# federicomegler/sq-learn

Measured on AMD Instinct MI355X. Metric: q-means fit samples/sec (Lloyd samples*iterations/s, delta-means + tomography noise), higher is better.
Workload: dtype fp32; 1 GPU; model=q-means k=1024 delta=0.5 (10000000 x 256 synthetic), global_batch=10000000, seq_len=256, parallelism=dp1

## Files before the change

sq_learn_amd/csrc/estep_f32.hip:

```cpp
#include "common.h"
#include "band.h"
#include "f16_tile.h"
#include "sq_api.h"

namespace sq {

constexpr int kMaxCand = 16;

#ifndef SQ_SPLIT_ACC_ALL
#define SQ_SPLIT_ACC_ALL 1
#endif
template <int KSD, int TOP = 2>
__global__ void __launch_bounds__(256, 1) estep_f32_kernel(
    const float* __restrict__ X, const _Float16* __restrict__ C, const float* __restrict__ xn,
    int* __restrict__ labels, float* __restrict__ mind, long long* __restrict__ ovf_rows,
    int* __restrict__ ovf_count, double* __restrict__ part, long long n, int k_pad, float alpha,
    float inv_alpha2, float delta_s, RngKey key, long long row_offset, int ovf_cap,
    const long long* __restrict__ rlist, const int* __restrict__ rcount,
    const float* __restrict__ cmax2_p, long long* __restrict__ mrows, int* __restrict__ mcand,
    int* __restrict__ multi_count, unsigned char* __restrict__ xflag, long long mcap) {
  const float Cm = cmax2_p ? sqrtf(*cmax2_p) * (1.0f + 0x1p-16f) : 0.0f;
  constexpr bool SPLIT_ACC = SQ_SPLIT_ACC_ALL || TOP == 3;
  constexpr float kEps3 =
      SPLIT_ACC ? (3.0f * 0x1p-22f + (KSD * 16 + 18.0f) * 0x1p-24f + 2.0f * KSD * 16 * 0x1p-34f) *
// ... 386 lines not shown
constexpr int kStampWaves = 8192;
constexpr int kStampN = 12;
__device__ unsigned long long g_x64_stamps[kStampWaves * kStampN];
#define SQ_STAMP_NOW() __builtin_amdgcn_s_memtime()
#endif

template <int KSD>
using X64Ring = TileRing<KSD, kX64Waves>;

template <int KSD>
struct X64RowSets {
  static constexpr int value = KSD <= 16 ? 2 : 1;
};
constexpr int kX64Pfd = 2;

template <int KSD, int RS>
__global__ void __launch_bounds__(kX64Waves * 64) estep_x64_kernel(
    const _Float16* __restrict__ Xh, const float* __restrict__ X, const _Float16* __restrict__ C,
    const float* __restrict__ Cm, const float* __restrict__ xn, const float* __restrict__ cmax2_p,
    int* __restrict__ labels, float* __restrict__ mind, long long* __restrict__ dense_rows,
    int* __restrict__ dense_count, long long* __restrict__ mrows, int* __restrict__ mcand,
    int* __restrict__ multi_count, long long n, int k_pad, float alpha, float delta_s,
    RngKey key, long long row_offset, int dense_cap, int qbits, const long long* __restrict__ rlist,
    const int* __restrict__ rcount, float* __restrict__ ub, float* __restrict__ lb,
    int* __restrict__ mflag) {
  constexpr int NW = kX64Waves;
  constexpr int DX = KSD * 16;
  using Ring = X64Ring<KSD>;
  constexpr int KT = Ring::KT, NS = Ring::NS, SK = Ring::SK, RING = Ring::RING;
  constexpr int ROWS = NW * 32 * RS;
  extern __shared__ __attribute__((aligned(16))) unsigned char smem[];
  auto buf = [&](int g) -> unsigned char* { return Ring::buf(smem, g); };
  int* cand_all = reinterpret_cast<int*>(smem + Ring::BYTES);
  int* cnt_all = cand_all + NW * RS * 32 * kMaxCand;

  const int tid = threadIdx.x;
  const int lane = tid & 63;
  const int wave = __builtin_amdgcn_readfirstlane(tid >> 6);
  const int r32 = lane & 31;
  const int half = lane >> 5;
  const int n_tiles = k_pad / kTileN;
  const long long ne = rlist ? min((long long)*rcount, n) : n;
  auto row_at = [&](long long pos) -> long long {
    const long long q = pos < ne ? pos : ne - 1;
    return rlist ? rlist[q] : q;
  };
  const long long nblk = (ne + ROWS - 1) / ROWS;
  long long blk = blockIdx.x;
  if (blk >= nblk) return;
  const uint32_t qmask = (1u << qbits) - 1u;
  const uint32_t keep = ~qmask;
  const float Ch = 2.0f * sqrtf(*cmax2_p) * (1.0f + 0x1p-16f);
  const float pack_rel = ldexpf(1.0f, qbits - 23) + 0x1p-15f;
  const float sub_rel = 0x1p-21f * sqrtf((float)DX);

  auto stage = [&](int U) { Ring::stage(C, smem, U, n_tiles); };

  f16x8 ah[RS][KSD];
  auto load_a = [&](long long b) {
    sq::load_a(ah, half, [&](int st) {
      return Xh + (size_t)row_at(b * ROWS + (wave * RS + st) * 32 + r32) * DX;
    });
  };
  const f16x8 aug = aug_frag(half);
  const int rl_own = acc_row(r32 >> 1, half);
  float xn_cur[RS], xn_nxt[RS];
  auto load_xn = [&](long long b, float (&dst)[RS]) {
#pragma unroll
    for (int st = 0; st < RS; ++st) dst[st] = xn[row_at(b * ROWS + (wave * RS + st) * 32 + rl_own)];
  };

  float m1[RS][16], m2[RS][16], m3[RS][16];
  const int lane_off = f16op::lane_off(half, r32);
  auto ins = [&](int st, int i, float v, uint32_t q) {
    const float p = and_or(v, keep, q);
    const float a1 = m1[st][i], a2 = m2[st][i];
    m3[st][i] = vmed3(a2, p, m3[st][i]);
    m2[st][i] = vmed3(a1, p, a2);
    m1[st][i] = vmin(a1, p);
  };
  typedef f32x16 Acc[RS][2];
  auto sub_step = [&](auto S_, const unsigned char* cur, Acc& acc, const Acc& o, int t_prev,
                      bool do_epi) {
    constexpr int S = decltype(S_)::value;
// ... 55 lines not shown
#endif
  };

  int U = 0;
  auto tile = [&](Acc& acc, const Acc& o, int t_prev, bool do_epi) {
#pragma unroll
    for (int st = 0; st < RS; ++st) acc[st][0] = acc[st][1] = (f32x16){0};
    static_for<NS>([&](auto S_) {
      stage(U + RING - 1);
      sub_step(S_, buf(U), acc, o, t_prev, do_epi);
      sync_tile();
      ++U;
    });
  };

  stage(0);
  stage(1);
  load_a(blk);
  load_xn(blk, xn_cur);
  asm volatile("s_waitcnt vmcnt(0)" ::: "memory");
  __builtin_amdgcn_s_barrier();

  for (; blk < nblk; blk += gridDim.x) {
#pragma unroll
    for (int st = 0; st < RS; ++st)
#pragma unroll
      for (int i = 0; i < 16; ++i) m1[st][i] = m2[st][i] = m3[st][i] = __builtin_inff();
    if constexpr (RS == 1) {
      Acc pA, pB;
      tile(pA, pA, 0, false);
      int t = 0;
      while (true) {
        if (t + 1 >= n_tiles) {
          load_a(blk + gridDim.x);
          load_xn(blk + gridDim.x, xn_nxt);
          epi_all(pA, t);
          break;
        }
        tile(pB, pA, t, true);
        ++t;
        if (t + 1 >= n_tiles) {
          load_a(blk + gridDim.x);
          load_xn(blk + gridDim.x, xn_nxt);
          epi_all(pB, t);
          break;
        }
        tile(pA, pB, t, true);
        ++t;
      }
    } else {
      f32x16 cA[RS], cB[RS];
      constexpr int PFD = kX64Pfd;
      f16x8 bq[PFD + 1];
      static_assert(NS == 1, "row sets need whole tiles per LDS slot");
#if SQ_X64_STAMP
      const unsigned long long sw0 = SQ_STAMP_NOW();
      st_first = true;
      ++st_blocks;
#endif
      for (int t = 0; t < n_tiles; ++t) {
#if SQ_X64_STAMP
        const unsigned long long sg0 = SQ_STAMP_NOW();
#endif
        stage(U + RING - 1);
#if SQ_X64_STAMP
        st_stage += SQ_STAMP_NOW() - sg0;
#endif
        tile_prime<KT>(buf(U), lane_off, bq);
        half_pass<0>(buf(U), lane_off, ah, aug, bq, cA, cB, (uint32_t)(2 * t - 1), t > 0, ins);
        half_pass<1>(buf(U), lane_off, ah, aug, bq, cB, cA, (uint32_t)(2 * t), true, ins);
        sync_tile();
        ++U;
      }
#if SQ_X64_STAMP
      const unsigned long long sl0 = SQ_STAMP_NOW();
#endif
      load_a(blk + gridDim.x);
      load_xn(blk + gridDim.x, xn_nxt);
#if SQ_X64_STAMP
      st_aload += SQ_STAMP_NOW() - sl0;
#endif
      half_drain(cB, (uint32_t)(2 * n_tiles - 1), ins);
#if SQ_X64_STAMP
      st_sweep += SQ_STAMP_NOW() - sw0;
#endif
    }
#if SQ_X64_STAMP
    const unsigned long long sp0 = SQ_STAMP_NOW();
#endif

#pragma nounroll
    for (int st = 0; st < RS; ++st) {
#if SQ_X64_STAMP
    const unsigned long long sc0 = SQ_STAMP_NOW();
#endif
    const long long row0 = blk * ROWS + (wave * RS + st) * 32;
    int* cand = cand_all + (wave * RS + st) * 32 * kMaxCand;
    int* cnt = cnt_all + (wave * RS + st) * 32;
    float ms1[16], ms2[16], ms3[16];
#pragma unroll
    for (int i = 0; i < 16; ++i) {
      ms1[i] = m1[0][i]; ms2[i] = m2[0][i]; ms3[i] = m3[0][i];
#pragma unroll
      for (int o = 1; o < RS; ++o) {
        const float a1 = m1[o][i], a2 = m2[o][i], a3 = m3[o][i];
        ms1[i] = st == o ? a1 : ms1[i];
        ms2[i] = st == o ? a2 : ms2[i];
        ms3[i] = st == o ? a3 : ms3[i];
      }
    }

    auto row_min = [&](float (&R)[16]) -> float {
#pragma unroll
      for (int o = 16, c = 8; o >= 2; o >>= 1, c >>= 1) {
        const bool hi = (r32 & o) != 0;
#pragma unroll
        for (int j = 0; j < c; ++j) {
          const float lo_v = R[j], hi_v = R[c + j];
          const float keepv = hi ? hi_v : lo_v, sendv = hi ? lo_v : hi_v;
          R[j] = vmin(keepv, __shfl_xor(sendv, o, 64));
        }
      }
      return vmin(R[0], __shfl_xor(R[0], 1, 64));
    };
    float R[16];
#pragma unroll
    for (int i = 0; i < 16; ++i) R[i] = ms1[i];
    const float rmin = row_min(R);
    float xn_own = xn_cur[0];
#pragma unroll
    for (int o = 1; o < RS; ++o) xn_own = st == o ? xn_cur[o] : xn_own;
    const float xsv = alpha * sqrtf(xn_own) * (1.0f + 0x1p-16f);
    const float prod = xsv * Ch;
    const float mag = 0.25f * Ch * Ch + prod;
    const float E = 1.0625f * 0x1p-10f * prod + pack_rel * mag + sub_rel * (xsv + Ch);
    const float T_own = __uint_as_float(__float_as_uint(rmin) & keep) + delta_s + 2.0f * E;

#if SQ_X64_STAMP
    const unsigned long long sc1 = SQ_STAMP_NOW();
    st_rmin += sc1 - sc0;
#endif
    float nc[16];
    float Tr[16];
#pragma unroll
    for (int i = 0; i < 16; ++i) Tr[i] = __shfl(T_own, 32 * half + 2 * i, 64);
    int* const sink = cnt_all + NW * RS * 32 + wave * 64 + lane;
#pragma unroll
    for (int i = 0; i < 16; ++i) {
      const float T = Tr[i];
      nc[i] = ms1[i] > T ? ms1[i] : (ms2[i] > T ? ms2[i] : ms3[i]);
      const int rl = acc_row(i, half);
      auto jof = [&](float p) -> int {
        const uint32_t q = __float_as_uint(p) & qmask;
        return (int)((q >> 1) * kTileN + (q & 1u) * 32u) + r32;
      };
      const unsigned long long b1 = __ballot(ms1[i] <= T), b2 = __ballot(ms2[i] <= T);
      const unsigned long long b3 = __ballot(ms3[i] <= T);
      const uint32_t b1l = (uint32_t)b1, b1h = (uint32_t)(b1 >> 32);
      const uint32_t b2l = (uint32_t)b2, b2h = (uint32_t)(b2 >> 32);
      const int c1 = __popc(half ? b1h : b1l), c2 = __popc(half ? b2h : b2l);
      const bool d3 = (half ? (uint32_t)(b3 >> 32) : (uint32_t)b3) != 0u;
      const int s1 = (int)__builtin_amdgcn_mbcnt_hi(b1h, __builtin_amdgcn_mbcnt_lo(b1l, 0u)) -
                     (half ? __popc(b1l) : 0);
      const int s2 = c1 + (int)__builtin_amdgcn_mbcnt_hi(b2h, __builtin_amdgcn_mbcnt_lo(b2l, 0u)) -
                     (half ? __popc(b2l) : 0);
      *((ms1[i] <= T && s1 < kMaxCand) ? cand + rl * kMaxCand + s1 : sink) = jof(ms1[i]);
      *((ms2[i] <= T && s2 < kMaxCand) ? cand + rl * kMaxCand + s2 : sink) = jof(ms2[i]);
      *(r32 == 0 ? cnt + rl : sink) = c1 + c2 + (d3 ? kMaxCand + 1 : 0);
    }
#if SQ_X64_STAMP
    const unsigned long long sc2 = SQ_STAMP_NOW();
    st_cl += sc2 - sc1;
#endif
    float ub_own = 0.f, lb_own = 0.f;
    if (ub) {
      const float ncmin = row_min(nc);
      const float ia2 = 1.0f / (alpha * alpha);
      const float d1 = (__uint_as_float(__float_as_uint(rmin) & keep) + E) * ia2;
      const float d2 = (__uint_as_float(__float_as_uint(ncmin) & keep) - E) * ia2;
      const float marg = 0x1p-20f * (xn_own + fabsf(d1) + fabsf(d2));
      ub_own = sqrtf(fmaxf(xn_own + d1 + marg, 0.f)) * (1.0f + 0x1p-20f);
      lb_own = sqrtf(fmaxf(xn_own + d2 - marg, 0.f)) * (1.0f - 0x1p-20f);
    }
    asm volatile("s_waitcnt lgkmcnt(0)" ::: "memory");
    __builtin_amdgcn_wave_barrier();
#if SQ_X64_STAMP
    st_cand += SQ_STAMP_NOW() - sc0;
    st_ub += SQ_STAMP_NOW() - sc2;
#endif

    const bool valid = row0 + r32 < ne;
    const long long g = row_at(row0 + r32);
    if (ub) {
      const int src = ((r32 & 3) + 4 * ((r32 >> 3) & 3)) * 2 + 32 * ((r32 >> 2) & 1);
      const float u = __shfl(ub_own, src, 64), l = __shfl(lb_own, src, 64);
      if (valid && half == 0) {
        ub[g] = u;
        lb[g] = cnt[r32] <= kMaxCand ? l : 0.0f;
      }
    }
    const int c_r = cnt[r32];
    const bool dense = c_r > kMaxCand;
    const bool multi = valid && !dense && c_r >= 2;
    if (mflag && valid && half == 0 && !multi) mflag[g] = 0;
    if (valid && half == 0) {
      if (dense) {
        const int s = atomicAdd(dense_count, 1);
        if (s < dense_cap) dense_rows[s] = g;
        labels[g] = -1;
      } else if (c_r == 1) {
        labels[g] = cand[r32 * kMaxCand];
        mind[g] = -1.0f;
      }
    }
    const bool mrow = multi && half == 0;
    const unsigned long long mm = __ballot(mrow);
    const int nm = __popcll(mm);
    int mbase = 0;
    if (lane == 0 && nm) mbase = atomicAdd(multi_count, nm);
    mbase = __shfl(mbase, 0, 64);
    if (mrow) {
      const long long slot = (long long)mbase + __popcll(mm & ((1ull << lane) - 1ull));
      if (mflag) mflag[g] = slot < n ? 1 : 0;
      if (slot < n) {
        mrows[slot] = g;
        int* mc = mcand + g * (kMaxCand + 1);
        mc[0] = c_r;
        for (int c = 0; c < c_r; ++c) mc[1 + c] = cand[r32 * kMaxCand + c];
      } else {
        const int s2 = atomicAdd(dense_count, 1);
        if (s2 < dense_cap) dense_rows[s2] = g;
        labels[g] = -1;
      }
    }
    asm volatile("s_waitcnt lgkmcnt(0)" ::: "memory");
    __builtin_amdgcn_wave_barrier();
    }
#pragma unroll
    for (int st = 0; st < RS; ++st) xn_cur[st] = xn_nxt[st];
#if SQ_X64_STAMP
    st_post += SQ_STAMP_NOW() - sp0;
#endif
  }
  asm volatile("s_waitcnt vmcnt(0)" ::: "memory");
#if SQ_X64_STAMP
  const int sidx = blockIdx.x * NW + wave;
  if (lane == 0 && sidx < kStampWaves) {
    unsigned long long* o = g_x64_stamps + (size_t)sidx * kStampN;
    o[0] = SQ_STAMP_NOW() - st_t0; o[1] = st_sweep; o[2] = st_sync; o[3] = st_sync0;
    o[4] = st_post; o[5] = st_blocks; o[6] = st_stage; o[7] = st_cand; o[8] = st_aload;
    o[9] = st_rmin; o[10] = st_cl; o[11] = st_ub;
  }
#endif
}

constexpr int kBfLdsK = 2048;
template <int PER>
// ... 1130 lines not shown
    hipOccupancyMaxActiveBlocksPerMultiprocessor(&per_cu, (const void*)gap_screen_kernel<DX>, 256,
                                                 0);
    gres = (long long)(cus > 0 ? cus : 256) * (per_cu > 0 ? per_cu : 2);
  }
  const unsigned bgrid =
      grid_blocks > 0 ? (unsigned)grid_blocks : (unsigned)min(max(rblocks, 1LL), gres);
  hipLaunchKernelGGL(gap_screen_kernel<DX>, dim3(bgrid), dim3(256), 0, st, (const _Float16*)Xh,
                     (const float*)xn, mrec.mrows_b, mrec.count_b, mrec.dsh, mrec.dsh_stride,
                     mrec.dq, mrec.dsh_stride / DX * 8, inv_alpha, delta, (int*)labels, mrec.rec,
                     mrec.mflag, mrec.it_now, mrec.ring, max(1, mrec.ring / 2), (long long*)mrows,
                     (int*)multi_count, cap, mrec.n_done, mrec.mrows_mv, mrec.count_mv,
                     (float*)ydbg);
  return (int)hipGetLastError();
}

template <int KSD>
static int launch_estep_x64(const void* Xh, const void* X, const void* C, const void* Cm,
                            const void* xn, const void* cmax2, void* labels, void* mind,
                            void* dense_rows, void* dense_count, void* mrows, void* mcand,
                            void* multi_count, void* corr, long long n, int k_pad, float alpha,
                            float delta_s, double delta, RngKey key, long long row_offset,
                            int dense_cap, hipStream_t st, const void* rlist, const void* rcount,
                            void* ub, void* lb, void* mflag, void* xflag, int list_rs,
                            const MultiRec& mrec, bool defer_rows = false) {
  int qbits = 1;
  while ((1 << qbits) < 2 * (k_pad / kTileN)) ++qbits;
  auto go = [&](auto RS_) {
    constexpr int RS = decltype(RS_)::value;
    constexpr int NW = kX64Waves;
    const size_t lds =
        (size_t)X64Ring<KSD>::BYTES + (size_t)NW * RS * 32 * (kMaxCand + 1) * 4 +
        (size_t)NW * 64 * 4;
    auto kern = estep_x64_kernel<KSD, RS>;
    static bool attr = false;
    if (!attr) {
      hipFuncSetAttribute((const void*)kern, hipFuncAttributeMaxDynamicSharedMemorySize,
                          160 * 1024);
      attr = true;
    }
    static int resident = 0;
    if (resident == 0) resident = resident_blocks((const void*)kern, NW * 64, lds);
    const long long nblk = (n + NW * 32 * RS - 1) / (NW * 32 * RS);
    const unsigned grid = (unsigned)(nblk < resident && !rlist ? nblk : resident);
    hipLaunchKernelGGL(kern, dim3(grid), dim3(NW * 64), lds, st, (const _Float16*)Xh,
                       (const float*)X, (const _Float16*)C, (const float*)Cm, (const float*)xn,
                       (const float*)cmax2, (int*)labels, (float*)mind, (long long*)dense_rows,
                       (int*)dense_count, (long long*)mrows, (int*)mcand, (int*)multi_count, n,
                       k_pad, alpha, delta_s, key, row_offset, dense_cap, qbits,
                       (const long long*)rlist, (const int*)rcount, (float*)ub, (float*)lb,
                       (int*)mflag);
  };
  static const bool list_rs1 = [] {
    const char* e = getenv("SQ_X64_LIST_RS1");
    return !(e && e[0] == '0');
  }();
  if (rlist && (list_rs == 1 || (list_rs == 0 && list_rs1)))
    go(std::integral_constant<int, 1>{});
  else
    go(std::integral_constant<int, X64RowSets<KSD>::value>{});
  int rc = (int)hipGetLastError();
  if (rc) return rc;
  const long long rblocks = (n / 16 + 63) / 64;
  const unsigned rgrid = (unsigned)(rblocks < 4096 ? (rblocks > 0 ? rblocks : 1) : 4096);
  if (xflag && mrec.rec && ub) {
    if constexpr (KSD * 16 % 128 == 0) {
      rc = launch_gap_screen<KSD * 16>(Xh, xn, mrec, 1.0f / alpha, (float)delta, labels, mrows,
                                       multi_count, n, rblocks, 0, nullptr, st);
      if (rc) return rc;
    }
  }
  if (xflag) {
    static int sgrid = 0, sil = 0;
    if (sgrid == 0) {
      const char* ei = getenv("SQ_SCREEN_IL");
// ... 132 lines not shown
                               row_offset, cap, st, rlist, rcount, ub, lb, mflag, xflag,         \
                               list_rs, mrec);                                                   \
    if (rc) return rc;                                                                           \
    rc = sq_rows_f64(X, d_pad, Cm, d_pad, d_pad, k, dense_rows, cnt + 1, 0, n, labels, mind,      \
                     corr, ub, delta, k0, k1, s0, s1, row_offset, (int)fgrid, stream);           \
    break;
    CASE(24) CASE(32) CASE(40) CASE(48) CASE(56) CASE(64)
#undef CASE
    default:
      return (int)hipErrorInvalidValue;
  }
  if (rc) return rc;
  return (int)hipGetLastError();
}

int sq_gap_screen(const void* Xh, const void* xn, const void* mrows_b, const void* count_b,
                  const void* dsh, const void* dq, long long dsh_stride, int ring, double alpha,
                  double delta, void* labels, void* rec, void* rec_mflag, int it_now, void* mrows,
                  void* multi_count, void* n_done, void* mrows_mv, void* count_mv, long long n,
                  int d_pad, int grid_blocks, void* ydbg, void* stream) {
  if ((mrows_mv != nullptr) != (count_mv != nullptr)) return (int)hipErrorInvalidValue;
  if (!Xh || !xn || !mrows_b || !count_b || !dsh || !dq || !labels || !rec || !rec_mflag ||
      !mrows || !multi_count || it_now < 1 || ring < 2 || ring > 16 || grid_blocks < 0)
    return (int)hipErrorInvalidValue;
  int aexp = 0;
  if (!(alpha > 0.0) || frexp(alpha, &aexp) != 0.5) return (int)hipErrorInvalidValue;
  if (n <= 0) return 0;
  const MultiRec mrec{(GapRec*)rec, (int*)rec_mflag, it_now, it_now, ring, (const _Float16*)dsh,
                      (const float*)dq, dsh_stride, (long long*)mrows_b, (int*)count_b,
                      (int*)n_done, (long long*)mrows_mv, (int*)count_mv};
// ... 57 lines not shown
```

sq_learn_amd/csrc/module.cpp:

```cpp
#define PY_SSIZE_T_CLEAN
#include <Python.h>
#include <hip/hip_runtime.h>

#include <array>
#include <cstdint>
#include <tuple>

#define SQ_API __attribute__((weak))
#include "sq_api.h"

template <class T, char C>
struct Scalar {
  using store = T;
  static constexpr char fmt = C;
  static T get(T v) { return v; }
};
template <class T> struct Slot;
template <> struct Slot<int> : Scalar<int, 'i'> {};
template <> struct Slot<long long> : Scalar<long long, 'L'> {};
template <> struct Slot<double> : Scalar<double, 'd'> {};
template <> struct Slot<float> : Scalar<float, 'f'> {};
template <> struct Slot<unsigned> : Scalar<unsigned, 'I'> {};
template <> struct Slot<unsigned long long> : Scalar<unsigned long long, 'K'> {};
template <class T>
// ... 184 lines not shown
    SQ_FN(sp_logit_multi, NOGIL, "CSR multinomial logistic loss and residual"),
    SQ_FN(sp_logit_bin, NOGIL, "CSR binary logistic loss and residual"),
    SQ_FN(sp_matvec, NOGIL, "CSR x fp64 vector product over row segments"),
    {nullptr, nullptr, 0, nullptr}};

static PyMethodDef gram_methods[] = {
    SQ_FN(sp_gram, 0, "CSR x CSR kernel matrix through an inverted index"),
    SQ_FN(sp_gram_matvec, 0, "CSR x CSR kernel matrix applied to vectors, never formed"),
    {nullptr, nullptr, 0, nullptr}};

static PyMethodDef mu_methods[] = {
    SQ_FN(sp_mu_row_waves, VALUE, "row partials of the CSR mu(A) kernel"),
    SQ_FN(sp_mu_sums, 0, "mu(A) power sums of a (centred) CSR matrix (fp64)"),
    {nullptr, nullptr, 0, nullptr}};

static struct PyModuleDef moddef ={PyModuleDef_HEAD_INIT, "_C",
                                    "sq_learn_amd native HIP kernels (gfx950)", -1, methods};
static struct PyModuleDef lda_moddef = {PyModuleDef_HEAD_INIT, "sq_learn_amd._C.lda",
                                        "latent Dirichlet allocation kernels (splda.hip)", -1,
                                        lda_methods};
static struct PyModuleDef nmf_moddef = {PyModuleDef_HEAD_INIT, "sq_learn_amd._C.nmf",
                                        "non-negative matrix factorisation kernels (spnmf.hip)",
                                        -1, nmf_methods};
static struct PyModuleDef logistic_moddef = {PyModuleDef_HEAD_INIT, "sq_learn_amd._C.logistic",
                                             "logistic-regression loss kernels (splogit.hip)", -1,
                                             logistic_methods};
static struct PyModuleDef gram_moddef = {PyModuleDef_HEAD_INIT, "sq_learn_amd._C.gram",
                                         "sparse kernel-matrix kernels (spgram.hip)", -1,
                                         gram_methods};
static struct PyModuleDef mu_moddef = {PyModuleDef_HEAD_INIT, "sq_learn_amd._C.mu",
                                       "sparse mu(A) power-sum kernels (spmu.hip)", -1,
                                       mu_methods};

static bool add_submodule(PyObject* m, const char* name, PyModuleDef* def) {
  PyObject* sub = PyModule_Create(def);
  if (!sub || PyModule_AddObject(m, name, sub) < 0) {
    Py_XDECREF(sub);
    return false;
  }
  return true;
}

PyMODINIT_FUNC PyInit__C(void) {
  PyObject* m = PyModule_Create(&moddef);
  if (!m) return nullptr;
  if (!add_submodule(m, "lda", &lda_moddef) || !add_submodule(m, "nmf", &nmf_moddef) ||
      !add_submodule(m, "logistic", &logistic_moddef) ||
      !add_submodule(m, "gram", &gram_moddef) || !add_submodule(m, "mu", &mu_moddef)) {
    Py_DECREF(m);
    return nullptr;
  }
  return m;
}
```

sq_learn_amd/csrc/sq_api.h:

```cpp
#pragma once

#ifndef SQ_API
#define SQ_API
#endif

extern "C" {

SQ_API int sq_trunc_normal_add(void* x, int dtype, long long n, double b, unsigned k0, unsigned k1,
                               unsigned s0, unsigned s1, unsigned long long offset, void* stream);
SQ_API int sq_philox_normal(void* out, int dtype, long long n, double mean, double stdv,
                            unsigned k0, unsigned k1, unsigned s0, unsigned s1,
                            unsigned long long offset, void* stream);
SQ_API int sq_philox_uniform(void* out, long long n, unsigned k0, unsigned k1, unsigned s0,
                             unsigned s1, unsigned long long offset, void* stream);
SQ_API int sq_ae_batch(const void* a, const void* eps, void* out, long long n, int Q, unsigned k0,
                       unsigned k1, unsigned s0, unsigned s1, unsigned long long offset,
                       void* stream);
SQ_API int sq_pe_batch(const void* omega, const void* m, void* out, long long n, unsigned k0,
                       unsigned k1, unsigned s0, unsigned s1, unsigned long long offset,
                       void* stream);

SQ_API int sq_tomography(const void* V, int r, int d, const void* sched, int T, int mode,
                         const void* first, void* err, void* out, int norm_inf, unsigned k0,
                         unsigned k1, unsigned s0, unsigned s1, long long row_offset, void* stream,
// ... 248 lines not shown
                        void* ovf_rows, void* ovf_count, void* part, int part_cap, void* inertia,
                        long long n, int d_pad, int k_pad, double alpha, double delta, unsigned k0,
                        unsigned k1, unsigned s0, unsigned s1, long long row_offset, int ovf_cap,
                        void* stream);
SQ_API int sq_estep_x64(const void* Xh, const void* X, const void* C, const void* Cm,
                        const void* xn, const void* cmax2, void* labels, void* mind,
                        void* dense_rows, void* ovf_rows, void* mrows, void* mcand, void* corr,
                        void* rlist, void* rcount, void* ub, void* lb, void* mflag, void* xflag,
                        void* counts, void* part, int part_cap, long long n, int d, int d_pad,
                        int k, int k_pad, double alpha, double delta, unsigned k0, unsigned k1,
                        unsigned s0, unsigned s1, long long row_offset, int list_rs, void* stream,
                        void* rec, void* rec_mflag, int it_now, int it_lo, int ring,
                        const void* dsh, const void* dq, long long dsh_stride, void* mrows_b,
                        void* count_b, void* n_done, void* mrows_mv, void* count_mv,
                        void* ovf2_rows, void* ovf2_count);
SQ_API int sq_gap_screen(const void* Xh, const void* xn, const void* mrows_b, const void* count_b,
                         const void* dsh, const void* dq, long long dsh_stride, int ring,
                         double alpha, double delta, void* labels, void* rec, void* rec_mflag,
                         int it_now, void* mrows, void* multi_count, void* n_done, void* mrows_mv,
                         void* count_mv, long long n, int d_pad, int grid_blocks, void* ydbg,
                         void* stream);
SQ_API int sq_x64_stamps(void* host, int n_waves);
SQ_API int sq_x64_stamps_clear();
SQ_API int sq_fill_mind(const void* X, int ldx, const void* Cm, int d, const void* labels,
                        void* mind, long long n, void* stream);
SQ_API int sq_sum_f32(const void* v, long long n, void* part, int extra, void* out, void* stream);
SQ_API int sq_centers_f16_operand(const void* Cm, void* op, int k, int d, int d_pad, int k_pad,
                                  double alpha, void* stream);

SQ_API int sq_rows_f64(const void* X, long long ldx, const void* C, long long ldc, int d, int k,
// ... 17 lines not shown
```

sq_learn_amd/models/cluster/_lloyd.py:

```python

import math
import os

import torch

from ...runtime.rng import RngKey
from ...ops import kmeans as K
from ...ops import linalg as L
from ...ops.random import trunc_normal_add_
from ...ops.failure import failure_inject_
from ...ops import _native as nat
from ...parallel.comm import Comm
from ...utils import tracing


class _HostScalars:

    __slots__ = ("host", "event", "sink")

    def __init__(self, host, event, sink=None):
        self.host, self.event, self.sink = host, event, sink

    def tolist(self):
        self.event.synchronize()
# ... 239 lines not shown
        self._ipe_buffers()
        self._ipe_lab[self._ipe_cur].copy_(t.to(self.device).to(torch.int32))
        self._ipe_hint_valid = bool((t >= 0).all())
        if getattr(self, "_ipe16", None) is not None:
            self._ipe16.invalidate_bounds()

    def _ipe_buffers(self):
        if getattr(self, "_ipe_lab", None) is None:
            self._ipe_lab = [torch.full((self.n,), -1, dtype=torch.int32, device=self.device)
                             for _ in range(2)]
            self._ipe_cur = 0
            self._ipe_xn = self.xn.float().contiguous()

    def _list_rs(self):
        force = os.environ.get("SQ_LIST_RS")
        if force is not None:
            return int(force)
        kf = self._kept_frac
        return 2 if (kf is None or kf > 0.3) else 0

    def _records_epoch(self):
        if getattr(self, "mrec", None) is not None:
            self._rit += 2
            self._rlo = self._rit

    def restore_tensors(self, d):
        self._pending = None
        self.inc_valid = False
        self.bounds_valid = False
        self._records_epoch()
        if self.fast and self.C_op is not None and "C_op" in d:
            self.C_op.copy_(d["C_op"].to(self.device))
        elif self.fast and self.C_op is None and "C_bf16" in d:
            self.C_bf16.copy_(d["C_bf16"].to(self.device))
# ... 545 lines not shown
```

sq_learn_amd/ops/kmeans.py:

```python

import math
import os
from typing import NamedTuple

import numpy as np

import torch

from ..runtime.rng import RngKey, philox4x32, MASK32
from . import _native as nat
from .random import amplitude_estimation_batch

FAST_D = (16, 32, 64, 128, 256)
X64_D = FAST_D + (384, 512, 640, 768, 896, 1024)
X64_MAX_K = 16384
BIG = 3.0e38


def pad_features(d):
    for f in X64_D:
        if d <= f:
            return f
    return ((d + 15) // 16) * 16

# ... 670 lines not shown
                           xn.data_ptr(), cmax2.data_ptr(), buf.labels.data_ptr(),
                           buf.mind.data_ptr(), buf.dense_rows.data_ptr(), buf.ovf_rows.data_ptr(),
                           buf.multi_rows.data_ptr(), buf.multi_cand.data_ptr(),
                           0 if buf.corr is None else buf.corr.data_ptr(),
                           0 if rows is None else rows[0].data_ptr(),
                           0 if rows is None else rows[1].data_ptr(),
                           0 if bounds is None else bounds[0].data_ptr(),
                           0 if bounds is None else bounds[1].data_ptr(),
                           0 if bounds is None else buf.mflag.data_ptr(),
                           buf.exact_flag.data_ptr() if screen else 0,
                           buf.counts.data_ptr(), buf.inertia_part.data_ptr(), int(buf.part_cap),
                           n, d_pad, d_pad, k, k_pad, float(alpha), float(delta), key.k0, key.k1,
                           key.s0, key.s1, int(row_offset), int(list_rs), st,
                           *(records if records is not None else (0,) * 13), *ovf2)
    return buf.labels, buf.mind


def fill_mind_native(Xf, C_master, labels, mind):
    n, ldx = Xf.shape
    nat.native().fill_mind(Xf.data_ptr(), ldx, C_master.data_ptr(), C_master.shape[1],
                           labels.data_ptr(), mind.data_ptr(), n, nat.stream_handle(Xf.device))


def sum_f32_native(v, n, part, out, extra=0):
    assert part.numel() >= 512 + extra and part.dtype == torch.float64 and extra >= 0
    nat.native().sum_f32(v.data_ptr(), int(n), part.data_ptr(), int(extra), out.data_ptr(),
                         nat.stream_handle(v.device))


KMPP_BOUND_MAX_DQ = 2048
# ... 569 lines not shown
```

Baseline: 16.72 billion samples*iter/s.

## Pair list-mode row rounds across grid strides in x64 E-step kernel

```diff
diff --git a/sq_learn_amd/csrc/estep_f32.hip b/sq_learn_amd/csrc/estep_f32.hip
--- a/sq_learn_amd/csrc/estep_f32.hip
+++ b/sq_learn_amd/csrc/estep_f32.hip
@@ -424,7 +424,7 @@
 };
 constexpr int kX64Pfd = 2;
 
-template <int KSD, int RS>
+template <int KSD, int RS, bool PAIR = false>
 __global__ void __launch_bounds__(kX64Waves * 64) estep_x64_kernel(
     const _Float16* __restrict__ Xh, const float* __restrict__ X, const _Float16* __restrict__ C,
     const float* __restrict__ Cm, const float* __restrict__ xn, const float* __restrict__ cmax2_p,
@@ -439,6 +439,8 @@
   using Ring = X64Ring<KSD>;
   constexpr int KT = Ring::KT, NS = Ring::NS, SK = Ring::SK, RING = Ring::RING;
   constexpr int ROWS = NW * 32 * RS;
+  constexpr int RROWS = NW * 32;
+  static_assert(!PAIR || (RS == 2 && NS == 1), "rounds are paired two at a time, whole tiles per slot");
   extern __shared__ __attribute__((aligned(16))) unsigned char smem[];
   auto buf = [&](int g) -> unsigned char* { return Ring::buf(smem, g); };
   int* cand_all = reinterpret_cast<int*>(smem + Ring::BYTES);
@@ -455,7 +457,10 @@
     const long long q = pos < ne ? pos : ne - 1;
     return rlist ? rlist[q] : q;
   };
-  const long long nblk = (ne + ROWS - 1) / ROWS;
+  const long long nblk = PAIR ? (ne + RROWS - 1) / RROWS : (ne + ROWS - 1) / ROWS;
+  auto pair_pos = [&](long long b, int st) -> long long {
+    return (b + (long long)st * gridDim.x) * RROWS + wave * 32;
+  };
   long long blk = blockIdx.x;
   if (blk >= nblk) return;
   const uint32_t qmask = (1u << qbits) - 1u;
@@ -469,7 +474,8 @@
   f16x8 ah[RS][KSD];
   auto load_a = [&](long long b) {
     sq::load_a(ah, half, [&](int st) {
-      return Xh + (size_t)row_at(b * ROWS + (wave * RS + st) * 32 + r32) * DX;
+      return Xh + (size_t)row_at(PAIR ? pair_pos(b, st) + r32
+                                      : b * ROWS + (wave * RS + st) * 32 + r32) * DX;
     });
   };
   const f16x8 aug = aug_frag(half);
@@ -477,7 +483,9 @@
   float xn_cur[RS], xn_nxt[RS];
   auto load_xn = [&](long long b, float (&dst)[RS]) {
 #pragma unroll
-    for (int st = 0; st < RS; ++st) dst[st] = xn[row_at(b * ROWS + (wave * RS + st) * 32 + rl_own)];
+    for (int st = 0; st < RS; ++st)
+      dst[st] = xn[row_at(PAIR ? pair_pos(b, st) + rl_own
+                               : b * ROWS + (wave * RS + st) * 32 + rl_own)];
   };
 
   float m1[RS][16], m2[RS][16], m3[RS][16];
@@ -563,6 +571,45 @@
     });
   };
 
+  auto tile_one = [&](auto& acc, const auto& o, int t_prev, bool do_epi) {
+    acc[0] = acc[1] = (f32x16){0};
+    stage(U + RING - 1);
+    const uint32_t q0 = (uint32_t)(t_prev * 2), q1 = q0 + 1u;
+    const unsigned char* hb = buf(U) + lane_off;
+    f16x8 b0[2], b1[2];
+    b0[0] = ldb(hb + f16op::frag_off(0, 0));
+    b1[0] = ldb(hb + f16op::frag_off(1, 0));
+#pragma unroll
+    for (int ks = 0; ks < KT; ++ks) {
+      const int c = ks & 1, nx = c ^ 1;
+      if (ks + 1 < KT) {
+        b0[nx] = ldb(hb + f16op::frag_off(0, ks + 1));
+        b1[nx] = ldb(hb + f16op::frag_off(1, ks + 1));
+      }
+      const f16x8 A = ks < KSD ? ah[0][ks] : aug;
+      acc[0] = __builtin_amdgcn_mfma_f32_32x32x16_f16(A, b0[c], acc[0], 0, 0, 0);
+      acc[1] = __builtin_amdgcn_mfma_f32_32x32x16_f16(A, b1[c], acc[1], 0, 0, 0);
+      if (do_epi) {
+#pragma unroll
+        for (int e = (ks * 16) / KT; e < ((ks + 1) * 16) / KT; ++e) {
+          ins(0, e, o[0][e], q0);
+          ins(0, e, o[1][e], q1);
+        }
+      }
+      __builtin_amdgcn_sched_barrier(0);
+    }
+    sync_tile();
+    ++U;
+  };
+  auto epi_all_one = [&](const auto& o, int t_prev) {
+    const uint32_t q0 = (uint32_t)(t_prev * 2), q1 = q0 + 1u;
+#pragma unroll
+    for (int i = 0; i < 16; ++i) {
+      ins(0, i, o[0][i], q0);
+      ins(0, i, o[1][i], q1);
+    }
+  };
+
   stage(0);
   stage(1);
   load_a(blk);
@@ -570,226 +617,24 @@
   asm volatile("s_waitcnt vmcnt(0)" ::: "memory");
   __builtin_amdgcn_s_barrier();
 
-  for (; blk < nblk; blk += gridDim.x) {
-#pragma unroll
-    for (int st = 0; st < RS; ++st)
-#pragma unroll
-      for (int i = 0; i < 16; ++i) m1[st][i] = m2[st][i] = m3[st][i] = __builtin_inff();
-    if constexpr (RS == 1) {
-      Acc pA, pB;
-      tile(pA, pA, 0, false);
-      int t = 0;
-      while (true) {
-        if (t + 1 >= n_tiles) {
-          load_a(blk + gridDim.x);
-          load_xn(blk + gridDim.x, xn_nxt);
-          epi_all(pA, t);
-          break;
-        }
-        tile(pB, pA, t, true);
-        ++t;
-        if (t + 1 >= n_tiles) {
-          load_a(blk + gridDim.x);
-          load_xn(blk + gridDim.x, xn_nxt);
-          epi_all(pB, t);
-          break;
-        }
-        tile(pA, pB, t, true);
-        ++t;
-      }
-    } else {
-      f32x16 cA[RS], cB[RS];
-      constexpr int PFD = kX64Pfd;
-      f16x8 bq[PFD + 1];
-      static_assert(NS == 1, "row sets need whole tiles per LDS slot");
-#if SQ_X64_STAMP
-      const unsigned long long sw0 = SQ_STAMP_NOW();
-      st_first = true;
-      ++st_blocks;
-#endif
-      for (int t = 0; t < n_tiles; ++t) {
-#if SQ_X64_STAMP
-        const unsigned long long sg0 = SQ_STAMP_NOW();
-#endif
-        stage(U + RING - 1);
-#if SQ_X64_STAMP
-        st_stage += SQ_STAMP_NOW() - sg0;
-#endif
-        tile_prime<KT>(buf(U), lane_off, bq);
-        half_pass<0>(buf(U), lane_off, ah, aug, bq, cA, cB, (uint32_t)(2 * t - 1), t > 0, ins);
-        half_pass<1>(buf(U), lane_off, ah, aug, bq, cB, cA, (uint32_t)(2 * t), true, ins);
-        sync_tile();
-        ++U;
-      }
-#if SQ_X64_STAMP
-      const unsigned long long sl0 = SQ_STAMP_NOW();
-#endif
-      load_a(blk + gridDim.x);
-      load_xn(blk + gridDim.x, xn_nxt);
-#if SQ_X64_STAMP
-      st_aload += SQ_STAMP_NOW() - sl0;
-#endif
-      half_drain(cB, (uint32_t)(2 * n_tiles - 1), ins);
-#if SQ_X64_STAMP
-      st_sweep += SQ_STAMP_NOW() - sw0;
-#endif
-    }
-#if SQ_X64_STAMP
-    const unsigned long long sp0 = SQ_STAMP_NOW();
-#endif
-
-#pragma nounroll
-    for (int st = 0; st < RS; ++st) {
-#if SQ_X64_STAMP
-    const unsigned long long sc0 = SQ_STAMP_NOW();
-#endif
-    const long long row0 = blk * ROWS + (wave * RS + st) * 32;
-    int* cand = cand_all + (wave * RS + st) * 32 * kMaxCand;
-    int* cnt = cnt_all + (wave * RS + st) * 32;
-    float ms1[16], ms2[16], ms3[16];
-#pragma unroll
-    for (int i = 0; i < 16; ++i) {
-      ms1[i] = m1[0][i]; ms2[i] = m2[0][i]; ms3[i] = m3[0][i];
-#pragma unroll
-      for (int o = 1; o < RS; ++o) {
-        const float a1 = m1[o][i], a2 = m2[o][i], a3 = m3[o][i];
-        ms1[i] = st == o ? a1 : ms1[i];
-        ms2[i] = st == o ? a2 : ms2[i];
-        ms3[i] = st == o ? a3 : ms3[i];
-      }
-    }
-
-    auto row_min = [&](float (&R)[16]) -> float {
-#pragma unroll
-      for (int o = 16, c = 8; o >= 2; o >>= 1, c >>= 1) {
-        const bool hi = (r32 & o) != 0;
-#pragma unroll
-        for (int j = 0; j < c; ++j) {
-          const float lo_v = R[j], hi_v = R[c + j];
-          const float keepv = hi ? hi_v : lo_v, sendv = hi ? lo_v : hi_v;
-          R[j] = vmin(keepv, __shfl_xor(sendv, o, 64));
-        }
-      }
-      return vmin(R[0], __shfl_xor(R[0], 1, 64));
-    };
-    float R[16];
-#pragma unroll
-    for (int i = 0; i < 16; ++i) R[i] = ms1[i];
-    const float rmin = row_min(R);
-    float xn_own = xn_cur[0];
-#pragma unroll
-    for (int o = 1; o < RS; ++o) xn_own = st == o ? xn_cur[o] : xn_own;
-    const float xsv = alpha * sqrtf(xn_own) * (1.0f + 0x1p-16f);
-    const float prod = xsv * Ch;
-    const float mag = 0.25f * Ch * Ch + prod;
-    const float E = 1.0625f * 0x1p-10f * prod + pack_rel * mag + sub_rel * (xsv + Ch);
-    const float T_own = __uint_as_float(__float_as_uint(rmin) & keep) + delta_s + 2.0f * E;
-
-#if SQ_X64_STAMP
-    const unsigned long long sc1 = SQ_STAMP_NOW();
-    st_rmin += sc1 - sc0;
-#endif
-    float nc[16];
-    float Tr[16];
-#pragma unroll
-    for (int i = 0; i < 16; ++i) Tr[i] = __shfl(T_own, 32 * half + 2 * i, 64);
-    int* const sink = cnt_all + NW * RS * 32 + wave * 64 + lane;
-#pragma unroll
-    for (int i = 0; i < 16; ++i) {
-      const float T = Tr[i];
-      nc[i] = ms1[i] > T ? ms1[i] : (ms2[i] > T ? ms2[i] : ms3[i]);
-      const int rl = acc_row(i, half);
-      auto jof = [&](float p) -> int {
-        const uint32_t q = __float_as_uint(p) & qmask;
-        return (int)((q >> 1) * kTileN + (q & 1u) * 32u) + r32;
-      };
-      const unsigned long long b1 = __ballot(ms1[i] <= T), b2 = __ballot(ms2[i] <= T);
-      const unsigned long long b3 = __ballot(ms3[i] <= T);
-      const uint32_t b1l = (uint32_t)b1, b1h = (uint32_t)(b1 >> 32);
-      const uint32_t b2l = (uint32_t)b2, b2h = (uint32_t)(b2 >> 32);
-      const int c1 = __popc(half ? b1h : b1l), c2 = __popc(half ? b2h : b2l);
-      const bool d3 = (half ? (uint32_t)(b3 >> 32) : (uint32_t)b3) != 0u;
-      const int s1 = (int)__builtin_amdgcn_mbcnt_hi(b1h, __builtin_amdgcn_mbcnt_lo(b1l, 0u)) -
-                     (half ? __popc(b1l) : 0);
-      const int s2 = c1 + (int)__builtin_amdgcn_mbcnt_hi(b2h, __builtin_amdgcn_mbcnt_lo(b2l, 0u)) -
-                     (half ? __popc(b2l) : 0);
-      *((ms1[i] <= T && s1 < kMaxCand) ? cand + rl * kMaxCand + s1 : sink) = jof(ms1[i]);
-      *((ms2[i] <= T && s2 < kMaxCand) ? cand + rl * kMaxCand + s2 : sink) = jof(ms2[i]);
-      *(r32 == 0 ? cnt + rl : sink) = c1 + c2 + (d3 ? kMaxCand + 1 : 0);
-    }
-#if SQ_X64_STAMP
-    const unsigned long long sc2 = SQ_STAMP_NOW();
-    st_cl += sc2 - sc1;
-#endif
-    float ub_own = 0.f, lb_own = 0.f;
-    if (ub) {
-      const float ncmin = row_min(nc);
-      const float ia2 = 1.0f / (alpha * alpha);
-      const float d1 = (__uint_as_float(__float_as_uint(rmin) & keep) + E) * ia2;
-      const float d2 = (__uint_as_float(__float_as_uint(ncmin) & keep) - E) * ia2;
-      const float marg = 0x1p-20f * (xn_own + fabsf(d1) + fabsf(d2));
-      ub_own = sqrtf(fmaxf(xn_own + d1 + marg, 0.f)) * (1.0f + 0x1p-20f);
-      lb_own = sqrtf(fmaxf(xn_own + d2 - marg, 0.f)) * (1.0f - 0x1p-20f);
-    }
-    asm volatile("s_waitcnt lgkmcnt(0)" ::: "memory");
-    __builtin_amdgcn_wave_barrier();
-#if SQ_X64_STAMP
-    st_cand += SQ_STAMP_NOW() - sc0;
-    st_ub += SQ_STAMP_NOW() - sc2;
-#endif
-
-    const bool valid = row0 + r32 < ne;
-    const long long g = row_at(row0 + r32);
-    if (ub) {
-      const int src = ((r32 & 3) + 4 * ((r32 >> 3) & 3)) * 2 + 32 * ((r32 >> 2) & 1);
-      const float u = __shfl(ub_own, src, 64), l = __shfl(lb_own, src, 64);
-      if (valid && half == 0) {
-        ub[g] = u;
-        lb[g] = cnt[r32] <= kMaxCand ? l : 0.0f;
-      }
-    }
-    const int c_r = cnt[r32];
-    const bool dense = c_r > kMaxCand;
-    const bool multi = valid && !dense && c_r >= 2;
-    if (mflag && valid && half == 0 && !multi) mflag[g] = 0;
-    if (valid && half == 0) {
-      if (dense) {
-        const int s = atomicAdd(dense_count, 1);
-        if (s < dense_cap) dense_rows[s] = g;
-        labels[g] = -1;
-      } else if (c_r == 1) {
-        labels[g] = cand[r32 * kMaxCand];
-        mind[g] = -1.0f;
-      }
-    }
-    const bool mrow = multi && half == 0;
-    const unsigned long long mm = __ballot(mrow);
-    const int nm = __popcll(mm);
-    int mbase = 0;
-    if (lane == 0 && nm) mbase = atomicAdd(multi_count, nm);
-    mbase = __shfl(mbase, 0, 64);
-    if (mrow) {
-      const long long slot = (long long)mbase + __popcll(mm & ((1ull << lane) - 1ull));
-      if (mflag) mflag[g] = slot < n ? 1 : 0;
-      if (slot < n) {
-        mrows[slot] = g;
-        int* mc = mcand + g * (kMaxCand + 1);
-        mc[0] = c_r;
-        for (int c = 0; c < c_r; ++c) mc[1 + c] = cand[r32 * kMaxCand + c];
-      } else {
-        const int s2 = atomicAdd(dense_count, 1);
-        if (s2 < dense_cap) dense_rows[s2] = g;
-        labels[g] = -1;
-      }
-    }
-    asm volatile("s_waitcnt lgkmcnt(0)" ::: "memory");
-    __builtin_amdgcn_wave_barrier();
-    }
-#pragma unroll
-    for (int st = 0; st < RS; ++st) xn_cur[st] = xn_nxt[st];
-#if SQ_X64_STAMP
-    st_post += SQ_STAMP_NOW() - sp0;
-#endif
+  int one_set = 1;
+  if constexpr (PAIR) asm volatile("" : "+s"(one_set));
+  if constexpr (!PAIR) {
+    constexpr bool ONE = false;
+    for (; blk < nblk; blk += gridDim.x) {
+#include "estep_x64_pass.h"
+    }
+  } else {
+    {
+      constexpr bool ONE = false;
+      for (; blk + gridDim.x < nblk; blk += 2LL * gridDim.x) {
+#include "estep_x64_pass.h"
+      }
+    }
+    if (blk < nblk) {
+      constexpr bool ONE = true;
+#include "estep_x64_pass.h"
+    }
   }
   asm volatile("s_waitcnt vmcnt(0)" ::: "memory");
 #if SQ_X64_STAMP
@@ -1950,6 +1795,12 @@
   return (int)hipGetLastError();
 }
 
+template <int KSD, int RS>
+static constexpr size_t x64_lds_bytes() {
+  return (size_t)X64Ring<KSD>::BYTES + (size_t)kX64Waves * RS * 32 * (kMaxCand + 1) * 4 +
+         (size_t)kX64Waves * 64 * 4;
+}
+
 template <int KSD>
 static int launch_estep_x64(const void* Xh, const void* X, const void* C, const void* Cm,
                             const void* xn, const void* cmax2, void* labels, void* mind,
@@ -1961,13 +1812,12 @@
                             const MultiRec& mrec, bool defer_rows = false) {
   int qbits = 1;
   while ((1 << qbits) < 2 * (k_pad / kTileN)) ++qbits;
-  auto go = [&](auto RS_) {
+  auto go = [&](auto RS_, auto PAIR_) {
     constexpr int RS = decltype(RS_)::value;
+    constexpr bool PAIR = decltype(PAIR_)::value;
     constexpr int NW = kX64Waves;
-    const size_t lds =
-        (size_t)X64Ring<KSD>::BYTES + (size_t)NW * RS * 32 * (kMaxCand + 1) * 4 +
-        (size_t)NW * 64 * 4;
-    auto kern = estep_x64_kernel<KSD, RS>;
+    const size_t lds = x64_lds_bytes<KSD, RS>();
+    auto kern = estep_x64_kernel<KSD, RS, PAIR>;
     static bool attr = false;
     if (!attr) {
       hipFuncSetAttribute((const void*)kern, hipFuncAttributeMaxDynamicSharedMemorySize,
@@ -1990,10 +1840,13 @@
     const char* e = getenv("SQ_X64_LIST_RS1");
     return !(e && e[0] == '0');
   }();
-  if (rlist && (list_rs == 1 || (list_rs == 0 && list_rs1)))
-    go(std::integral_constant<int, 1>{});
+  constexpr bool kPairs = X64RowSets<KSD>::value == 2;
+  if (rlist && list_rs == 0 && list_rs1 && kPairs)
+    go(std::integral_constant<int, X64RowSets<KSD>::value>{}, std::integral_constant<bool, kPairs>{});
+  else if (rlist && (list_rs == 1 || (list_rs == 0 && list_rs1)))
+    go(std::integral_constant<int, 1>{}, std::false_type{});
   else
-    go(std::integral_constant<int, X64RowSets<KSD>::value>{});
+    go(std::integral_constant<int, X64RowSets<KSD>::value>{}, std::false_type{});
   int rc = (int)hipGetLastError();
   if (rc) return rc;
   const long long rblocks = (n / 16 + 63) / 64;
@@ -2156,6 +2009,22 @@
   return (int)hipGetLastError();
 }
 
+int sq_x64_list_wave_slots(int d_pad) {
+  switch (d_pad) {
+#define CASE(KSD)                                                                                \
+  case KSD * 16: {                                                                               \
+    constexpr bool P = X64RowSets<KSD>::value == 2;                                              \
+    const void* kern = (const void*)estep_x64_kernel<KSD, P ? 2 : 1, P>;                         \
+    hipFuncSetAttribute(kern, hipFuncAttributeMaxDynamicSharedMemorySize, 160 * 1024);           \
+    return resident_blocks(kern, kX64Waves * 64, x64_lds_bytes<KSD, P ? 2 : 1>()) * kX64Waves;   \
+  }
+    CASE(1) CASE(2) CASE(4) CASE(8) CASE(16) CASE(24) CASE(32) CASE(40) CASE(48) CASE(56) CASE(64)
+#undef CASE
+    default:
+      return 0;
+  }
+}
+
 int sq_gap_screen(const void* Xh, const void* xn, const void* mrows_b, const void* count_b,
                   const void* dsh, const void* dq, long long dsh_stride, int ring, double alpha,
                   double delta, void* labels, void* rec, void* rec_mflag, int it_now, void* mrows,
diff --git a/sq_learn_amd/csrc/estep_x64_pass.h b/sq_learn_amd/csrc/estep_x64_pass.h
--- /dev/null
+++ b/sq_learn_amd/csrc/estep_x64_pass.h
@@ -0,0 +1,239 @@
+#pragma unroll
+    for (int st = 0; st < RS; ++st)
+#pragma unroll
+      for (int i = 0; i < 16; ++i) m1[st][i] = m2[st][i] = m3[st][i] = __builtin_inff();
+    if constexpr (RS == 1) {
+      Acc pA, pB;
+      tile(pA, pA, 0, false);
+      int t = 0;
+      while (true) {
+        if (t + 1 >= n_tiles) {
+          load_a(blk + gridDim.x);
+          load_xn(blk + gridDim.x, xn_nxt);
+          epi_all(pA, t);
+          break;
+        }
+        tile(pB, pA, t, true);
+        ++t;
+        if (t + 1 >= n_tiles) {
+          load_a(blk + gridDim.x);
+          load_xn(blk + gridDim.x, xn_nxt);
+          epi_all(pB, t);
+          break;
+        }
+        tile(pA, pB, t, true);
+        ++t;
+      }
+    } else if constexpr (ONE) {
+      f32x16 pA[2], pB[2];
+      tile_one(pA, pA, 0, false);
+      int t = 0;
+      while (true) {
+        if (t + 1 >= n_tiles) {
+          epi_all_one(pA, t);
+          break;
+        }
+        tile_one(pB, pA, t, true);
+        ++t;
+        if (t + 1 >= n_tiles) {
+          epi_all_one(pB, t);
+          break;
+        }
+        tile_one(pA, pB, t, true);
+        ++t;
+      }
+    } else {
+      f32x16 cA[RS], cB[RS];
+      constexpr int PFD = kX64Pfd;
+      f16x8 bq[PFD + 1];
+      static_assert(NS == 1, "row sets need whole tiles per LDS slot");
+#if SQ_X64_STAMP
+      const unsigned long long sw0 = SQ_STAMP_NOW();
+      st_first = true;
+      ++st_blocks;
+#endif
+      for (int t = 0; t < n_tiles; ++t) {
+#if SQ_X64_STAMP
+        const unsigned long long sg0 = SQ_STAMP_NOW();
+#endif
+        stage(U + RING - 1);
+#if SQ_X64_STAMP
+        st_stage += SQ_STAMP_NOW() - sg0;
+#endif
+        tile_prime<KT>(buf(U), lane_off, bq);
+        half_pass<0>(buf(U), lane_off, ah, aug, bq, cA, cB, (uint32_t)(2 * t - 1), t > 0, ins);
+        half_pass<1>(buf(U), lane_off, ah, aug, bq, cB, cA, (uint32_t)(2 * t), true, ins);
+        sync_tile();
+        ++U;
+      }
+#if SQ_X64_STAMP
+      const unsigned long long sl0 = SQ_STAMP_NOW();
+#endif
+      load_a(PAIR ? blk + 2LL * gridDim.x : blk + gridDim.x);
+      load_xn(PAIR ? blk + 2LL * gridDim.x : blk + gridDim.x, xn_nxt);
+#if SQ_X64_STAMP
+      st_aload += SQ_STAMP_NOW() - sl0;
+#endif
+      half_drain(cB, (uint32_t)(2 * n_tiles - 1), ins);
+#if SQ_X64_STAMP
+      st_sweep += SQ_STAMP_NOW() - sw0;
+#endif
+    }
+#if SQ_X64_STAMP
+    const unsigned long long sp0 = SQ_STAMP_NOW();
+#endif
+
+#pragma nounroll
+    for (int st = 0; st < (ONE ? one_set : RS); ++st) {
+#if SQ_X64_STAMP
+    const unsigned long long sc0 = SQ_STAMP_NOW();
+#endif
+    const long long row0 = PAIR ? pair_pos(blk, st) : blk * ROWS + (wave * RS + st) * 32;
+    int* cand = cand_all + (wave * RS + st) * 32 * kMaxCand;
+    int* cnt = cnt_all + (wave * RS + st) * 32;
+    float ms1[16], ms2[16], ms3[16];
+#pragma unroll
+    for (int i = 0; i < 16; ++i) {
+      ms1[i] = m1[0][i]; ms2[i] = m2[0][i]; ms3[i] = m3[0][i];
+#pragma unroll
+      for (int o = 1; o < RS; ++o) {
+        const float a1 = m1[o][i], a2 = m2[o][i], a3 = m3[o][i];
+        ms1[i] = st == o ? a1 : ms1[i];
+        ms2[i] = st == o ? a2 : ms2[i];
+        ms3[i] = st == o ? a3 : ms3[i];
+      }
+    }
+
+    auto row_min = [&](float (&R)[16]) -> float {
+#pragma unroll
+      for (int o = 16, c = 8; o >= 2; o >>= 1, c >>= 1) {
+        const bool hi = (r32 & o) != 0;
+#pragma unroll
+        for (int j = 0; j < c; ++j) {
+          const float lo_v = R[j], hi_v = R[c + j];
+          const float keepv = hi ? hi_v : lo_v, sendv = hi ? lo_v : hi_v;
+          R[j] = vmin(keepv, __shfl_xor(sendv, o, 64));
+        }
+      }
+      return vmin(R[0], __shfl_xor(R[0], 1, 64));
+    };
+    float R[16];
+#pragma unroll
+    for (int i = 0; i < 16; ++i) R[i] = ms1[i];
+    const float rmin = row_min(R);
+    float xn_own = xn_cur[0];
+#pragma unroll
+    for (int o = 1; o < RS; ++o) xn_own = st == o ? xn_cur[o] : xn_own;
+    const float xsv = alpha * sqrtf(xn_own) * (1.0f + 0x1p-16f);
+    const float prod = xsv * Ch;
+    const float mag = 0.25f * Ch * Ch + prod;
+    const float E = 1.0625f * 0x1p-10f * prod + pack_rel * mag + sub_rel * (xsv + Ch);
+    const float T_own = __uint_as_float(__float_as_uint(rmin) & keep) + delta_s + 2.0f * E;
+
+#if SQ_X64_STAMP
+    const unsigned long long sc1 = SQ_STAMP_NOW();
+    st_rmin += sc1 - sc0;
+#endif
+    float nc[16];
+    float Tr[16];
+#pragma unroll
+    for (int i = 0; i < 16; ++i) Tr[i] = __shfl(T_own, 32 * half + 2 * i, 64);
+    int* const sink = cnt_all + NW * RS * 32 + wave * 64 + lane;
+#pragma unroll
+    for (int i = 0; i < 16; ++i) {
+      const float T = Tr[i];
+      nc[i] = ms1[i] > T ? ms1[i] : (ms2[i] > T ? ms2[i] : ms3[i]);
+      const int rl = acc_row(i, half);
+      auto jof = [&](float p) -> int {
+        const uint32_t q = __float_as_uint(p) & qmask;
+        return (int)((q >> 1) * kTileN + (q & 1u) * 32u) + r32;
+      };
+      const unsigned long long b1 = __ballot(ms1[i] <= T), b2 = __ballot(ms2[i] <= T);
+      const unsigned long long b3 = __ballot(ms3[i] <= T);
+      const uint32_t b1l = (uint32_t)b1, b1h = (uint32_t)(b1 >> 32);
+      const uint32_t b2l = (uint32_t)b2, b2h = (uint32_t)(b2 >> 32);
+      const int c1 = __popc(half ? b1h : b1l), c2 = __popc(half ? b2h : b2l);
+      const bool d3 = (half ? (uint32_t)(b3 >> 32) : (uint32_t)b3) != 0u;
+      const int s1 = (int)__builtin_amdgcn_mbcnt_hi(b1h, __builtin_amdgcn_mbcnt_lo(b1l, 0u)) -
+                     (half ? __popc(b1l) : 0);
+      const int s2 = c1 + (int)__builtin_amdgcn_mbcnt_hi(b2h, __builtin_amdgcn_mbcnt_lo(b2l, 0u)) -
+                     (half ? __popc(b2l) : 0);
+      *((ms1[i] <= T && s1 < kMaxCand) ? cand + rl * kMaxCand + s1 : sink) = jof(ms1[i]);
+      *((ms2[i] <= T && s2 < kMaxCand) ? cand + rl * kMaxCand + s2 : sink) = jof(ms2[i]);
+      *(r32 == 0 ? cnt + rl : sink) = c1 + c2 + (d3 ? kMaxCand + 1 : 0);
+    }
+#if SQ_X64_STAMP
+    const unsigned long long sc2 = SQ_STAMP_NOW();
+    st_cl += sc2 - sc1;
+#endif
+    float ub_own = 0.f, lb_own = 0.f;
+    if (ub) {
+      const float ncmin = row_min(nc);
+      const float ia2 = 1.0f / (alpha * alpha);
+      const float d1 = (__uint_as_float(__float_as_uint(rmin) & keep) + E) * ia2;
+      const float d2 = (__uint_as_float(__float_as_uint(ncmin) & keep) - E) * ia2;
+      const float marg = 0x1p-20f * (xn_own + fabsf(d1) + fabsf(d2));
+      ub_own = sqrtf(fmaxf(xn_own + d1 + marg, 0.f)) * (1.0f + 0x1p-20f);
+      lb_own = sqrtf(fmaxf(xn_own + d2 - marg, 0.f)) * (1.0f - 0x1p-20f);
+    }
+    asm volatile("s_waitcnt lgkmcnt(0)" ::: "memory");
+    __builtin_amdgcn_wave_barrier();
+#if SQ_X64_STAMP
+    st_cand += SQ_STAMP_NOW() - sc0;
+    st_ub += SQ_STAMP_NOW() - sc2;
+#endif
+
+    const bool valid = row0 + r32 < ne;
+    const long long g = row_at(row0 + r32);
+    if (ub) {
+      const int src = ((r32 & 3) + 4 * ((r32 >> 3) & 3)) * 2 + 32 * ((r32 >> 2) & 1);
+      const float u = __shfl(ub_own, src, 64), l = __shfl(lb_own, src, 64);
+      if (valid && half == 0) {
+        ub[g] = u;
+        lb[g] = cnt[r32] <= kMaxCand ? l : 0.0f;
+      }
+    }
+    const int c_r = cnt[r32];
+    const bool dense = c_r > kMaxCand;
+    const bool multi = valid && !dense && c_r >= 2;
+    if (mflag && valid && half == 0 && !multi) mflag[g] = 0;
+    if (valid && half == 0) {
+      if (dense) {
+        const int s = atomicAdd(dense_count, 1);
+        if (s < dense_cap) dense_rows[s] = g;
+        labels[g] = -1;
+      } else if (c_r == 1) {
+        labels[g] = cand[r32 * kMaxCand];
+        mind[g] = -1.0f;
+      }
+    }
+    const bool mrow = multi && half == 0;
+    const unsigned long long mm = __ballot(mrow);
+    const int nm = __popcll(mm);
+    int mbase = 0;
+    if (lane == 0 && nm) mbase = atomicAdd(multi_count, nm);
+    mbase = __shfl(mbase, 0, 64);
+    if (mrow) {
+      const long long slot = (long long)mbase + __popcll(mm & ((1ull << lane) - 1ull));
+      if (mflag) mflag[g] = slot < n ? 1 : 0;
+      if (slot < n) {
+        mrows[slot] = g;
+        int* mc = mcand + g * (kMaxCand + 1);
+        mc[0] = c_r;
+        for (int c = 0; c < c_r; ++c) mc[1 + c] = cand[r32 * kMaxCand + c];
+      } else {
+        const int s2 = atomicAdd(dense_count, 1);
+        if (s2 < dense_cap) dense_rows[s2] = g;
+        labels[g] = -1;
+      }
+    }
+    asm volatile("s_waitcnt lgkmcnt(0)" ::: "memory");
+    __builtin_amdgcn_wave_barrier();
+    }
+    if constexpr (!ONE) {
+#pragma unroll
+    for (int st = 0; st < RS; ++st) xn_cur[st] = xn_nxt[st];
+    }
+#if SQ_X64_STAMP
+    st_post += SQ_STAMP_NOW() - sp0;
+#endif
diff --git a/sq_learn_amd/csrc/module.cpp b/sq_learn_amd/csrc/module.cpp
--- a/sq_learn_amd/csrc/module.cpp
+++ b/sq_learn_amd/csrc/module.cpp
@@ -222,6 +222,10 @@
     SQ_FN(sp_mu_sums, 0, "mu(A) power sums of a (centred) CSR matrix (fp64)"),
     {nullptr, nullptr, 0, nullptr}};
 
+static PyMethodDef lloyd_methods[] = {
+    SQ_FN(x64_list_wave_slots, VALUE, "wave slots of the list-mode filter sweep at d_pad"),
+    {nullptr, nullptr, 0, nullptr}};
+
 static struct PyModuleDef moddef ={PyModuleDef_HEAD_INIT, "_C",
                                     "sq_learn_amd native HIP kernels (gfx950)", -1, methods};
 static struct PyModuleDef lda_moddef = {PyModuleDef_HEAD_INIT, "sq_learn_amd._C.lda",
@@ -239,6 +243,9 @@
 static struct PyModuleDef mu_moddef = {PyModuleDef_HEAD_INIT, "sq_learn_amd._C.mu",
                                        "sparse mu(A) power-sum kernels (spmu.hip)", -1,
                                        mu_methods};
+static struct PyModuleDef lloyd_moddef = {PyModuleDef_HEAD_INIT, "sq_learn_amd._C.lloyd",
+                                          "Lloyd-step kernels (estep_f32.hip)", -1,
+                                          lloyd_methods};
 
 static bool add_submodule(PyObject* m, const char* name, PyModuleDef* def) {
   PyObject* sub = PyModule_Create(def);
@@ -254,7 +261,8 @@
   if (!m) return nullptr;
   if (!add_submodule(m, "lda", &lda_moddef) || !add_submodule(m, "nmf", &nmf_moddef) ||
       !add_submodule(m, "logistic", &logistic_moddef) ||
-      !add_submodule(m, "gram", &gram_moddef) || !add_submodule(m, "mu", &mu_moddef)) {
+      !add_submodule(m, "gram", &gram_moddef) || !add_submodule(m, "mu", &mu_moddef) ||
+      !add_submodule(m, "lloyd", &lloyd_moddef)) {
     Py_DECREF(m);
     return nullptr;
   }
diff --git a/sq_learn_amd/csrc/sq_api.h b/sq_learn_amd/csrc/sq_api.h
--- a/sq_learn_amd/csrc/sq_api.h
+++ b/sq_learn_amd/csrc/sq_api.h
@@ -286,6 +286,7 @@
                         const void* dsh, const void* dq, long long dsh_stride, void* mrows_b,
                         void* count_b, void* n_done, void* mrows_mv, void* count_mv,
                         void* ovf2_rows, void* ovf2_count);
+SQ_API int sq_x64_list_wave_slots(int d_pad);
 SQ_API int sq_gap_screen(const void* Xh, const void* xn, const void* mrows_b, const void* count_b,
                          const void* dsh, const void* dq, long long dsh_stride, int ring,
                          double alpha, double delta, void* labels, void* rec, void* rec_mflag,
diff --git a/sq_learn_amd/models/cluster/_lloyd.py b/sq_learn_amd/models/cluster/_lloyd.py
--- a/sq_learn_amd/models/cluster/_lloyd.py
+++ b/sq_learn_amd/models/cluster/_lloyd.py
@@ -277,10 +277,7 @@
 
     def _list_rs(self):
         force = os.environ.get("SQ_LIST_RS")
-        if force is not None:
-            return int(force)
-        kf = self._kept_frac
-        return 2 if (kf is None or kf > 0.3) else 0
+        return int(force) if force is not None else 0
 
     def _records_epoch(self):
         if getattr(self, "mrec", None) is not None:
diff --git a/sq_learn_amd/ops/kmeans.py b/sq_learn_amd/ops/kmeans.py
--- a/sq_learn_amd/ops/kmeans.py
+++ b/sq_learn_amd/ops/kmeans.py
@@ -708,6 +708,13 @@
                            key.s0, key.s1, int(row_offset), int(list_rs), st,
                            *(records if records is not None else (0,) * 13), *ovf2)
     return buf.labels, buf.mind
+
+
+def x64_list_wave_slots(d_pad):
+    w = int(nat.native().lloyd.x64_list_wave_slots(int(d_pad)))
+    if w <= 0:
+        raise ValueError(f"d_pad = {d_pad} is not a shape of the certified E-step")
+    return w
 
 
 def fill_mind_native(Xf, C_master, labels, mind):
```

Result: no change. 16.69 billion samples*iter/s (median of 2 runs) (-0.2%).
